# adrianstanea/UnitSpeech

Hardware: AMD Instinct MI355X
Metric: mel-frames/sec @ 50 diffusion steps, 80x1024 (higher is better)
Workload: dtype f32; 1 GPU; B=1 utterance(s)/GPU, 80x1024 mel, 50 diffusion steps, text+spk CFG (3 score evals/step), full-size decoder (119.1M params, synthetic weights), built-in Philox noise; batch_per_gpu=1, frames=1024, diffusion_steps=50, parallelism=utterance-sharded x1

## Files before the change

unitspeech_amd/csrc/attn.hip:

```cpp
#include "kernels.h"

namespace us {

typedef float f32x16 __attribute__((ext_vector_type(16)));
typedef float f32x4 __attribute__((ext_vector_type(4)));

constexpr int kChunk = 128;
constexpr int kQkvLd = 3 * kHidden;

__global__ __launch_bounds__(256) void attn_ctx_partial_kernel(const float* __restrict__ qkv, int n, float* __restrict__ part_ctx,
                                                               float* __restrict__ part_m, float* __restrict__ part_s, int nchunks) {
  const int b = blockIdx.y, chunk = blockIdx.x;
  const int lane = threadIdx.x & 63, h = threadIdx.x >> 6;
  const int c = lane & 31, hh = lane >> 5;
  const float* base = qkv + (long long)b * n * kQkvLd;
  const int r0 = chunk * kChunk;
  const float* kp = base + kHidden + h * kDimHead + c;
  const float* vp = base + 2 * kHidden + h * kDimHead + c;

  float kv[kChunk / 2];
  float m = -INFINITY;
#pragma unroll
  for (int j = 0; j < kChunk / 2; ++j) {
    int row = r0 + 2 * j + hh;
// ... 64 lines not shown
                                                              int per_split, float* __restrict__ ctx, float* __restrict__ split_ws) {
  const int b = blockIdx.x / kHeads, h = blockIdx.x % kHeads;
  const int d = threadIdx.x >> 5, e = threadIdx.x & 31;
  const float M = colM[(long long)b * kHidden + h * kDimHead + d], S = colS[(long long)b * kHidden + h * kDimHead + d];
  const int lo = blockIdx.y * per_split;
  int hi = lo + per_split;
  if (hi > nchunks) hi = nchunks;
  const float* pm = part_m + (long long)b * nchunks * kHidden + h * kDimHead + d;
  const float* pc = part_ctx + ((long long)b * nchunks * kHeads + h) * (kDimHead * kDimHead) + d * kDimHead + e;
  float acc0 = 0.f, acc1 = 0.f, acc2 = 0.f, acc3 = 0.f;
  int ch = lo;
  for (; ch + 4 <= hi; ch += 4) {
    float m0 = pm[(long long)ch * kHidden], m1 = pm[(long long)(ch + 1) * kHidden], m2 = pm[(long long)(ch + 2) * kHidden],
          m3 = pm[(long long)(ch + 3) * kHidden];
    float c0 = pc[(long long)ch * kHeads * 1024], c1 = pc[(long long)(ch + 1) * kHeads * 1024], c2 = pc[(long long)(ch + 2) * kHeads * 1024],
          c3 = pc[(long long)(ch + 3) * kHeads * 1024];
    acc0 = fmaf(expf(m0 - M), c0, acc0);
    acc1 = fmaf(expf(m1 - M), c1, acc1);
    acc2 = fmaf(expf(m2 - M), c2, acc2);
    acc3 = fmaf(expf(m3 - M), c3, acc3);
  }
  for (; ch < hi; ++ch) acc0 = fmaf(expf(pm[(long long)ch * kHidden] - M), pc[(long long)ch * kHeads * 1024], acc0);
  const float v = ((acc0 + acc1) + (acc2 + acc3)) / S;
  float* dst = (gridDim.y == 1 ? ctx : split_ws + (long long)blockIdx.y * gridDim.x * (kDimHead * kDimHead)) +
               ((long long)b * kHeads + h) * (kDimHead * kDimHead) + d * kDimHead + e;
  *dst = v;
}

__global__ __launch_bounds__(1024) void attn_ctx_reduce_kernel(const float* __restrict__ split_ws, int nsplit, long long slab,
                                                               float* __restrict__ ctx) {
  const long long i = blockIdx.x * 1024LL + threadIdx.x;
  float acc = split_ws[i];
  for (int k = 1; k < nsplit; ++k) acc += split_ws[i + k * slab];
  ctx[i] = acc;
}

hipError_t launch_attn_ctx_finalize(const float* part_ctx, const float* part_m, const float* part_s, int B, int nchunks,
                                    float* ctx, float* colM, float* colS, float* split_ws, hipStream_t s) {
  hipLaunchKernelGGL(attn_ctx_stats_kernel, dim3(B * kHeads), dim3(1024), 0, s, part_m, part_s, nchunks, colM, colS);
  int nsplit = (nchunks + 31) / 32;
  if (nsplit > kAttnMaxSplit) nsplit = kAttnMaxSplit;
  if (nsplit < 1 || !split_ws) nsplit = 1;
  const int per_split = (nchunks + nsplit - 1) / nsplit;
  nsplit = (nchunks + per_split - 1) / per_split;
  hipLaunchKernelGGL(attn_ctx_accum_kernel, dim3(B * kHeads, nsplit), dim3(1024), 0, s, part_ctx, part_m, colM, colS, nchunks, per_split, ctx,
                     split_ws);
  if (nsplit > 1)
    hipLaunchKernelGGL(attn_ctx_reduce_kernel, dim3(B * kHeads), dim3(1024), 0, s, split_ws, nsplit,
                       (long long)B * kHeads * kDimHead * kDimHead, ctx);
  return hipGetLastError();
}

__global__ __launch_bounds__(1024) void attn_merge_kernel(const float* __restrict__ part_ctx, const float* __restrict__ part_m,
                                                          const float* __restrict__ part_s, int nchunks, int per_range,
                                                          float* __restrict__ r_ctx, float* __restrict__ r_m, float* __restrict__ r_s) {
  __shared__ float s_m[64][kDimHead + 1];
  __shared__ float s_M[kDimHead], s_S[kDimHead];
  const int bh = blockIdx.y, b = bh / kHeads, h = bh % kHeads;
  const int d = threadIdx.x >> 5, e = threadIdx.x & 31;
  const int lo = blockIdx.x * per_range;
  const int hi = min(lo + per_range, nchunks);
  const float* pm = part_m + (long long)b * nchunks * kHidden + h * kDimHead;
  const float* ps = part_s + (long long)b * nchunks * kHidden + h * kDimHead;
  const float* pc = part_ctx + ((long long)b * nchunks * kHeads + h) * (kDimHead * kDimHead) + d * kDimHead + e;
  float M = -INFINITY;
  for (int ch = lo + d; ch < hi; ch += 32) M = fmaxf(M, pm[(long long)ch * kHidden + e]);
  s_m[d][e] = M;
  __syncthreads();
  if (d == 0) {
    float mm = s_m[0][e];
#pragma unroll
    for (int k = 1; k < 32; ++k) mm = fmaxf(mm, s_m[k][e]);
    s_M[e] = mm;
  }
  __syncthreads();
  {
    const float Mc = s_M[e];
    float S = 0.f;
    for (int ch = lo + d; ch < hi; ch += 32) S += ps[(long long)ch * kHidden + e] * expf(pm[(long long)ch * kHidden + e] - Mc);
    __syncthreads();
    s_m[d][e] = S;
    __syncthreads();
    if (d == 0) {
      float ss = 0.f;
#pragma unroll
      for (int k = 0; k < 32; ++k) ss += s_m[k][e];
      s_S[e] = ss;
    }
  }
  __syncthreads();
  const float Md = s_M[d];
  float acc0 = 0.f, acc1 = 0.f, acc2 = 0.f, acc3 = 0.f;
  for (int base = lo; base < hi; base += 64) {
    const int nb = min(64, hi - base);
    __syncthreads();
    for (int i = threadIdx.x; i < nb * kDimHead; i += 1024) {
      const int c = i >> 5, col = i & 31;
      s_m[c][col] = expf(pm[(long long)(base + c) * kHidden + col] - s_M[col]);
    }
    __syncthreads();
    int c = 0;
    for (; c + 8 <= nb; c += 8) {
      float v[8];
#pragma unroll
      for (int u = 0; u < 8; ++u) v[u] = pc[(long long)(base + c + u) * kHeads * 1024];
      acc0 = fmaf(s_m[c][d], v[0], acc0);     acc1 = fmaf(s_m[c + 1][d], v[1], acc1);
      acc2 = fmaf(s_m[c + 2][d], v[2], acc2); acc3 = fmaf(s_m[c + 3][d], v[3], acc3);
      acc0 = fmaf(s_m[c + 4][d], v[4], acc0); acc1 = fmaf(s_m[c + 5][d], v[5], acc1);
      acc2 = fmaf(s_m[c + 6][d], v[6], acc2); acc3 = fmaf(s_m[c + 7][d], v[7], acc3);
    }
    for (; c < nb; ++c) acc0 = fmaf(s_m[c][d], pc[(long long)(base + c) * kHeads * 1024], acc0);
  }
  (void)Md;
  const long long o = ((long long)blockIdx.x * gridDim.y + bh);
  r_ctx[o * 1024 + d * kDimHead + e] = (acc0 + acc1) + (acc2 + acc3);
  if (d == 0) { r_m[o * kDimHead + e] = s_M[e]; r_s[o * kDimHead + e] = s_S[e]; }
}

__global__ __launch_bounds__(1024) void attn_final_kernel(const float* __restrict__ r_ctx, const float* __restrict__ r_m,
                                                          const float* __restrict__ r_s, int nrange, float* __restrict__ ctx,
                                                          float* __restrict__ colM, float* __restrict__ colS, const float* __restrict__ wout,
                                                          float* __restrict__ weff, int C, int bk, int f16, unsigned* range_flag) {
  __shared__ float s_ctx[kDimHead][kDimHead + 1];
  __shared__ float s_w[16][kDimHead + 1];
  __shared__ float s_M[kDimHead], s_S[kDimHead];
  const int bh = blockIdx.x, b = bh / kHeads, h = bh % kHeads;
  const int d = threadIdx.x >> 5, e = threadIdx.x & 31;
  const int nbh = gridDim.x;
  const bool writer = blockIdx.y == 0;
  if (d == 0) {
    float M = -INFINITY;
    for (int r = 0; r < nrange; ++r) M = fmaxf(M, r_m[((long long)r * nbh + bh) * kDimHead + e]);
    float S = 0.f;
    for (int r = 0; r < nrange; ++r) {
      const float w = expf(r_m[((long long)r * nbh + bh) * kDimHead + e] - M);
      s_w[r][e] = w;
      S += r_s[((long long)r * nbh + bh) * kDimHead + e] * w;
    }
    s_M[e] = M; s_S[e] = S;
    if (writer) {
      colM[(long long)b * kHidden + h * kDimHead + e] = M;
      colS[(long long)b * kHidden + h * kDimHead + e] = S;
    }
  }
  __syncthreads();
  float acc = 0.f;
  for (int r = 0; r < nrange; ++r) acc = fmaf(s_w[r][d], r_ctx[((long long)r * nbh + bh) * 1024 + d * kDimHead + e], acc);
  const float v = acc / s_S[d];
  if (writer) ctx[((long long)b * kHeads + h) * 1024 + d * kDimHead + e] = v;
  if (!weff) return;
  s_ctx[d][e] = v;
  __syncthreads();
  const int dd = threadIdx.x & 31;
  bool over = false;
  const int co_end = min(C, ((int)blockIdx.y + 1) * 128);
  __shared__ float s_wo[128][kDimHead + 1];
  for (int i = threadIdx.x; i < 128 * kDimHead; i += 1024) {
    const int r = i >> 5, k = i & 31, co = blockIdx.y * 128 + r;
    s_wo[r][k] = co < C ? wout[(long long)co * kHidden + h * kDimHead + k] : 0.f;
  }
  __syncthreads();
  for (int co = blockIdx.y * 128 + (threadIdx.x >> 5); co < co_end; co += 32) {
    const float* w = s_wo[co - blockIdx.y * 128];
    float a2 = 0.f;
#pragma unroll
    for (int k = 0; k < kDimHead; ++k) a2 = fmaf(w[k], s_ctx[dd][k], a2);
    const int hd = h * kDimHead + dd;
    const long long o = (long long)b * C * kHidden + ((long long)(hd / bk) * C + co) * bk;
    if (!f16) {
      weff[o + hd % bk] = a2;
    } else {
      _Float16* w16 = reinterpret_cast<_Float16*>(weff + o);
      const int k = hd % 32;
      us_half hh_, ll_;
      split_f16x3(a2, hh_, ll_, over);
      w16[(k / 8) * 16 + k % 8] = hh_;
      w16[(k / 8) * 16 + 8 + k % 8] = ll_;
    }
  }
  range_report(range_flag, over, kRangeWeight);
}

hipError_t launch_attn_merge(const float* part_ctx, const float* part_m, const float* part_s, int B, int nchunks, float* ctx, float* colM,
                             float* colS, float* scratch, const float* wout, float* weff, int C, int bk, bool f16, hipStream_t s) {
  if (f16 && bk != 32) return hipErrorInvalidValue;
  int nrange = (nchunks + 63) / 64;
  if (nrange > kAttnMaxSplit) nrange = kAttnMaxSplit;
  if (nrange < 1) nrange = 1;
  const int per_range = (nchunks + nrange - 1) / nrange;
  nrange = (nchunks + per_range - 1) / per_range;
  const long long nbh = (long long)B * kHeads;
  float* r_ctx = scratch;
  float* r_m = r_ctx + (long long)kAttnMaxSplit * nbh * 1024;
  float* r_s = r_m + (long long)kAttnMaxSplit * nbh * kDimHead;
  hipLaunchKernelGGL(attn_merge_kernel, dim3(nrange, (unsigned)nbh), dim3(1024), 0, s, part_ctx, part_m, part_s, nchunks, per_range, r_ctx, r_m, r_s);
  hipLaunchKernelGGL(attn_final_kernel, dim3((unsigned)nbh, weff ? (unsigned)((C + 127) / 128) : 1u), dim3(1024), 0, s, r_ctx, r_m, r_s, nrange, ctx, colM, colS, wout, weff, C, bk,
                     f16 ? 1 : 0, current_range_flag());
  return hipGetLastError();
}

__global__ __launch_bounds__(256) void attn_wtotal_kernel(const float* __restrict__ ctx, const float* __restrict__ wout,
                                                          const float* __restrict__ wq, float* __restrict__ wtotal, int C, int bk, int f16,
                                                          unsigned* range_flag) {
  __shared__ __attribute__((aligned(16))) float s_T[kHidden][36];
  __shared__ float s_C[kHidden][33];
  __shared__ __attribute__((aligned(16))) float s_QW[kHidden * 36];
  const int b = blockIdx.y, k0 = blockIdx.x * 32, n0 = blockIdx.z * 32;
  const float* cx = ctx + (long long)b * kHeads * kDimHead * kDimHead;
  for (int i = threadIdx.x; i < kHidden * 32; i += 256) {
    s_C[i >> 5][i & 31] = cx[i];
    s_QW[(i >> 5) * 36 + (i & 31)] = wq[(long long)(i >> 5) * C + k0 + (i & 31)];
  }
  __syncthreads();
  for (int i = threadIdx.x; i < kHidden * 8; i += 256) {
    const int j = i >> 3, k4 = (i & 7) * 4;
    const int h = j / kDimHead, e = j % kDimHead;
    f32x4 acc = {0.f, 0.f, 0.f, 0.f};
#pragma unroll
    for (int d = 0; d < kDimHead; ++d) {
      const float c = s_C[h * kDimHead + d][e];
      const f32x4 q = *reinterpret_cast<const f32x4*>(&s_QW[(h * kDimHead + d) * 36 + k4]);
#pragma unroll
      for (int t = 0; t < 4; ++t) acc[t] = fmaf(c, q[t], acc[t]);
    }
    *reinterpret_cast<f32x4*>(&s_T[j][k4]) = acc;
  }
  __syncthreads();
  float* s_W = s_QW;
  for (int i = threadIdx.x; i < 32 * kHidden; i += 256) s_W[(i / kHidden) * (kHidden + 1) + i % kHidden] = wout[(long long)(n0 + i / kHidden) * kHidden + i % kHidden];
  __syncthreads();
  bool over = false;
  const int nl = threadIdx.x >> 3, g8 = threadIdx.x & 7;
  const int n = n0 + nl;
  f32x4 acc = {0.f, 0.f, 0.f, 0.f};
  for (int j = 0; j < kHidden; ++j) {
    const float wj = s_W[nl * (kHidden + 1) + j];
    const f32x4 tv = *reinterpret_cast<const f32x4*>(&s_T[j][g8 * 4]);
#pragma unroll
    for (int t = 0; t < 4; ++t) acc[t] = fmaf(wj, tv[t], acc[t]);
  }
  float* base = wtotal + (long long)b * C * C;
  if (f16) {
    typedef _Float16 half4_t __attribute__((ext_vector_type(4)));
    half4_t hi, lo;
#pragma unroll
    for (int t = 0; t < 4; ++t) {
      us_half h_, l_;
      split_f16x3(acc[t], h_, l_, over);
      hi[t] = h_;
      lo[t] = l_;
// ... 56 lines not shown
```

unitspeech_amd/csrc/decoder.hip:

```cpp
#include <hip/hip_runtime.h>

#include <cmath>
#include <cstdarg>
#include <cstdio>
#include <cstring>
#include <algorithm>
#include <map>
#include <memory>
#include <string>
#include <vector>

#include "../../include/unitspeech_hip.h"
#include "kernels.h"
#include "pack_f16.h"

using namespace us;

namespace {

thread_local std::string g_last_error;

struct DevBuf {
  float* p = nullptr;
  size_t n = 0;
// ... 42 lines not shown
  Slot *mlp_w, *mlp_b;
  ConvW c1, c2, res;
  Slot *g1, *b1, *g2, *b2;
  bool has_res = false;
  int index = 0;
};
struct AttnW {
  int dim, level;
  Slot* g;
  ConvW qkv;
  Slot *out_w, *out_b;
};
struct ResampleW {
  ConvW conv;
  int dim, level;
};

int pick_bk(int cin) { return (cin % 32 == 0) ? 32 : 16; }
constexpr const char* kWino4Default = "0,44,44,24";

}

namespace us {
void set_last_error(const char* msg) { g_last_error = msg ? msg : ""; }
}

struct us_decoder {
  us_config cfg{};
  int device = 0;
  std::vector<std::unique_ptr<Slot>> slots;
  std::map<std::string, Slot*> by_key;
  std::vector<int> C;
  struct Down { ResnetW r1, r2; AttnW a; bool has_ds; ResampleW ds; };
  struct Up { ResnetW r1, r2; AttnW a; ResampleW us; };
  std::vector<Down> downs;
  ResnetW mid1, mid2;
  AttnW mid_attn;
  std::vector<Up> ups;
  ConvW final_conv3;
  Slot *final_g, *final_b, *final_w1, *final_b1;
  Slot *text_uncon, *spk_uncon, *mlp0_w, *mlp0_b, *mlp2_w, *mlp2_b;
  int n_resnets = 0;
  int wino_min_level = 1;
  int wino4_level_form[8] = {0, 0, 0, 0, 0, 0, 0, 0};
  int wino_fuse = -1;
  bool wino_fuse_gn = true;
  int f16_tm = 0;
  int wgrad_side_streams = 1;
  std::vector<hipStream_t> wgrad_streams;
  std::vector<hipEvent_t> wgrad_events;
  bool training = false;
  float* zeros = nullptr;
  unsigned* range_flag = nullptr;
  unsigned* range_host = nullptr;
  bool exact = false;
  float* grad_scale = nullptr;
  CopyEnt* grad_tab_dev = nullptr;
  static constexpr size_t kLinJobs = 64;
  LinJob *lin_tab_dev = nullptr, *lin_tab_bwd_dev = nullptr;
  std::vector<CopyEnt> pending_copies;
  std::vector<PackJob> pending_packs;
  PackJob* pack_tab_dev = nullptr;
  static constexpr size_t kStageBytes = 64 << 10;
  CopyEnt* copy_tab_dev = nullptr;
  CopyEnt* copy_tab_host[4] = {nullptr, nullptr, nullptr, nullptr};
  static constexpr int kCaptureTabs = 32;
  size_t copy_tab_capture_bytes[kCaptureTabs] = {};
  CopyEnt* copy_tab_capture[kCaptureTabs] = {};
  int copy_tab_capture_used = 0;
  hipEvent_t copy_tab_ev[4] = {nullptr, nullptr, nullptr, nullptr};
  int copy_tab_i = 0;
  size_t copy_tab_cap = 0;
  std::map<uint64_t, std::shared_ptr<void>> tapes;
  uint64_t tape_serial = 0;
  static constexpr size_t kMaxTapes = 16;
  std::string err;

  struct ProfRec { hipEvent_t a, b; double flops; int kind; int f16 = 0; };
  bool prof_enabled = false;
  bool prof_active = false;
  std::vector<ProfRec> prof_pending;
  std::vector<hipEvent_t> prof_pool;
  double prof_conv_ms = 0, prof_conv_flops = 0, prof_eval_ms = 0;
  long long prof_conv_launches = 0, prof_evals = 0;
  double prof_f16_ms = 0, prof_f16_flops = 0;
  long long prof_f16_launches = 0;
  hipEvent_t prof_event() {
    if (!prof_pool.empty()) { hipEvent_t e = prof_pool.back(); prof_pool.pop_back(); return e; }
    hipEvent_t e = nullptr;
    (void)hipEventCreate(&e);
    return e;
  }

  int fail(int code, const char* fmt, ...) {
    char buf[512];
    va_list ap;
    va_start(ap, fmt);
    vsnprintf(buf, sizeof buf, fmt, ap);
    va_end(ap);
    err = buf;
    g_last_error = buf;
    return code;
  }

  Slot* add(const std::string& key, std::vector<int64_t> shape, Kind kind = Kind::RAW, int bk = 0) {
    slots.emplace_back(new Slot());
// ... 522 lines not shown
    g.stats = st1; g.gamma = r.g1->buf.p; g.beta = r.b1->buf.p; g.temb = tproj;
    g.mask = e.mask; g.mask_ld = e.T; g.mask_step = 1 << l; g.mask_bmod = e.Bm;
    CK(conv3x3_wino(e, r.c2, S1, r.cout, l, S2, r.cout, st2, &g));
  } else {
    if (direct_presplit(e, r.c2, r.cout, out_ld) && out != in) {
      CK(gn_apply(e, S1, l, r.cout, st1, r.g1, r.b1, tproj, nullptr, 0, false, true, out, r.cout, true));
      CK(conv3x3(e, r.c2, out, r.cout, l, S2, r.cout, st2, true));
    } else {
      CK(gn_apply(e, S1, l, r.cout, st1, r.g1, r.b1, tproj, nullptr, 0, false, true, S1, r.cout));
      CK(conv3x3(e, r.c2, S1, r.cout, l, S2, r.cout, st2));
    }
  }
  if (R) {
    CK(gn_apply(e, S2, l, r.cout, st2, r.g2, r.b2, nullptr, R, r.cout, false, mask_out, out, out_ld, false, split_out));
  } else if (r.has_res) {
    CK(gn_apply(e, S2, l, r.cout, st2, r.g2, r.b2, nullptr, nullptr, 0, false, false, out, out_ld));
    CK(conv1x1(e, r.res, in, in_ld, l, mask_out, out, out_ld, out, out_ld, nullptr, nullptr, 0, nullptr, in_split));
  } else {
    CK(gn_apply(e, S2, l, r.cout, st2, r.g2, r.b2, nullptr, in, in_ld, false, mask_out, out, out_ld, false, split_out));
  }
  return hipSuccess;
}

inline bool next_takes_split_copy(EvalCtx& e, const ResnetW& r2) {
  return !e.h->exact && !r2.has_res && !r2.first && direct_presplit(e, r2.c1, r2.c1.cin, r2.c1.cin) &&
         r2.c1.cin == r2.cout;
}

inline bool resnet_takes_split(EvalCtx& e, const ResnetW& r) {
  return !r.first && r.has_res && !(r.c1.w->wino.p && e.b->wino_v) && r.c1.w->direct_f16 && r.res.w->direct_f16;
}

hipError_t attention(EvalCtx& e, const AttnW& at, const float* in, int in_ld, float* out, int out_ld, bool out_split = false) {
  Buffers& b = *e.b;
  const int l = at.level;
  const int n = (e.h->cfg.n_feats >> l) * (e.T >> l);
  const int nch = attn_nchunks(n);
  float* qkv = b.QKV[l];
  int q_ld = 3 * kHidden;
  int nparts = nch;
  if (at.qkv.w->qkv_rows.p && at.qkv.w->q_raw.p && b.wtotal && l == 0 && at.dim <= kWtotalMaxC && at.dim % 32 == 0) {
    const int H = e.h->cfg.n_feats >> l, W = e.T >> l;
    const int nch64 = (n + 63) / 64;
    ConvArgs a = base_args(e, at.qkv, in, in_ld, H, W, qkv, kHidden, H, W);
    a.Cout = 2 * kHidden;
    a.wt_rows = 3 * kHidden;
    a.wt = at.qkv.w->qkv_rows.p + (size_t)kHidden * at.qkv.w->bk;
    a.ntaps = 1;
    a.set_tap(0, 0, 0, 0);
    a.attn_part_ctx = b.part_ctx; a.attn_part_m = b.part_m; a.attn_part_s = b.part_s; a.attn_nchunks = nch64;
    a.attn_q_cols = 0;
    CK(run_conv(e, a));
    const bool f16 = !e.h->exact;
    CK(launch_attn_merge(b.part_ctx, b.part_m, b.part_s, e.Bp, nch64, b.ctx, b.colM, b.colS, b.ctx_split, at.out_w->buf.p, nullptr, at.dim,
                         pick_bk(kHidden), f16, e.s));
    const int bkc = pick_bk(at.dim);
    CK(launch_attn_wtotal(b.ctx, at.out_w->buf.p, at.qkv.w->q_raw.p, b.wtotal, e.Bp, at.dim, bkc, f16, e.s));
    ConvW tot;
    tot.cin = at.dim; tot.cout = at.dim;
    Slot tmp;
    tmp.bk = bkc; tmp.buf.p = b.wtotal; tmp.direct_f16 = f16;
    tot.w = &tmp; tot.b = nullptr;
    return conv1x1(e, tot, in, in_ld, l, true, out, out_ld, in, in_ld, at.g->buf.p, b.wtotal, (long long)at.dim * at.dim, at.out_b->buf.p,
                   false, out_split);
  }
  if (at.qkv.w->qkv_rows.p) {
    const int H = e.h->cfg.n_feats >> l, W = e.T >> l;
    const int nch64 = (n + 63) / 64;
    q_ld = kHidden;
    ConvArgs a = base_args(e, at.qkv, in, in_ld, H, W, qkv, q_ld, H, W);
    a.wt = at.qkv.w->qkv_rows.p;
    a.ntaps = 1;
    a.set_tap(0, 0, 0, 0);
    a.attn_part_ctx = b.part_ctx; a.attn_part_m = b.part_m; a.attn_part_s = b.part_s; a.attn_nchunks = nch64;
    a.attn_q_cols = kHidden;
    CK(run_conv(e, a));
    nparts = nch64;
  } else {
    CK(conv1x1(e, at.qkv, in, in_ld, l, false, qkv, 3 * kHidden, nullptr, 0, nullptr, nullptr, 0, nullptr));
    CK(launch_attn_ctx_partial(qkv, e.Bp, n, b.part_ctx, b.part_m, b.part_s, nch, e.s));
  }
  const int bk = pick_bk(kHidden);
  const bool f16 = !e.h->exact;
  CK(launch_attn_merge(b.part_ctx, b.part_m, b.part_s, e.Bp, nparts, b.ctx, b.colM, b.colS, b.ctx_split, at.out_w->buf.p, b.weff, at.dim, bk,
                       f16, e.s));
  ConvW eff;
  eff.cin = kHidden; eff.cout = at.dim;
  Slot tmp;
  tmp.bk = bk; tmp.buf.p = b.weff; tmp.direct_f16 = f16;
  eff.w = &tmp; eff.b = nullptr;
  return conv1x1(e, eff, qkv, q_ld, l, true, out, out_ld, in, in_ld, at.g->buf.p, b.weff, (long long)at.dim * kHidden,
                 at.out_b->buf.p, false, out_split);
}

int upload_bytes(us_decoder* h, const void* src, size_t nbytes, void* dev, hipStream_t st);

inline int proj_jobs(us_decoder* h, std::vector<LinJob>& jobs, std::vector<const ResnetW*>& blocks) {
  jobs.clear();
  blocks.clear();
  int o0 = 0;
  auto add = [&](const ResnetW& r) {
    LinJob j;
    memset(&j, 0, sizeof j);
    j.W = r.mlp_w->buf.p; j.bias = r.mlp_b->buf.p; j.o0 = o0; j.cout = r.cout; j.out_ld = r.cout;
    jobs.push_back(j);
    blocks.push_back(&r);
    o0 += r.cout;
  };
  for (auto& d : h->downs) { add(d.r1); add(d.r2); }
  add(h->mid1); add(h->mid2);
  for (auto& u : h->ups) { add(u.r1); add(u.r2); }
  return o0;
}

hipError_t time_embedding(EvalCtx& e, const float* t, const float* spk) {
  us_decoder* h = e.h;
  Buffers& b = *e.b;
  const int dim = h->cfg.dim, S = h->cfg.spk_emb_dim, td = dim + S;
  CK(launch_pos_emb(t, b.posemb, e.Bp, dim, h->cfg.pe_scale, e.s));
  CK(launch_linear(b.posemb, dim, h->mlp0_w->buf.p, h->mlp0_b->buf.p, b.mlp_h, 4 * dim, e.Bp, dim, 4 * dim, false, e.s));
  CK(launch_linear(b.mlp_h, 4 * dim, h->mlp2_w->buf.p, h->mlp2_b->buf.p, b.temb, td, e.Bp, 4 * dim, dim, true, e.s));
  CK(launch_copy_rows(spk, S, e.Bp, b.temb + dim, td, e.Bp, S, e.s));
  std::vector<LinJob> jobs;
  std::vector<const ResnetW*> blocks;
  const int total = proj_jobs(h, jobs, blocks);
  if (h->lin_tab_dev && jobs.size() <= us_decoder::kLinJobs) {
    for (size_t i = 0; i < jobs.size(); ++i) jobs[i].out = b.tproj + b.tproj_off[blocks[i]->index];
    if (upload_bytes(h, jobs.data(), jobs.size() * sizeof(LinJob), h->lin_tab_dev, e.s) != US_OK) return hipErrorUnknown;
    return launch_linear_multi(h->lin_tab_dev, (int)jobs.size(), total, b.temb, td, e.Bp, td, true, e.s);
  }
  auto proj = [&](const ResnetW& r) {
    return launch_linear(b.temb, td, r.mlp_w->buf.p, r.mlp_b->buf.p, b.tproj + b.tproj_off[r.index], r.cout, e.Bp, td, r.cout, true,
                         e.s);
  };
  for (auto& d : h->downs) { CK(proj(d.r1)); CK(proj(d.r2)); }
  CK(proj(h->mid1)); CK(proj(h->mid2));
  for (auto& u : h->ups) { CK(proj(u.r1)); CK(proj(u.r2)); }
// ... 245 lines not shown
  if (h->cfg.n_feats % q != 0) return h->fail(US_EINVAL, "n_feats=%d is not divisible by %d", h->cfg.n_feats, q);
  return US_OK;
}

}

extern "C" {

int us_decoder_create(us_handle* out, const us_config* cfg) { return us_decoder_create_ex(out, cfg, 0u); }

int us_decoder_create_ex(us_handle* out, const us_config* cfg, unsigned flags) {
  if (!out || !cfg) { g_last_error = "null argument"; return US_EINVAL; }
  if (flags & ~(unsigned)US_CREATE_EXACT_FP32) { g_last_error = "unknown creation flag"; return US_EINVAL; }
  if (cfg->n_mults < 1 || cfg->n_mults > 6 || cfg->dim < 16 || cfg->dim % 16 != 0 || cfg->n_feats <= 0 || cfg->spk_emb_dim <= 0 ||
      cfg->spk_emb_dim % 4 != 0) {
    g_last_error = "unsupported configuration (dim must be a multiple of 16, 1 <= n_mults <= 6)";
    return US_EINVAL;
  }
  for (int i = 0; i < cfg->n_mults; ++i) {
    int c = cfg->dim * cfg->dim_mults[i];
    int cg = c / kGroups;
    if (cfg->dim_mults[i] < 1 || c % 16 != 0 || (cg & (cg - 1)) != 0) {
      g_last_error = "unsupported dim_mults (channels/8 must be a power of two)";
      return US_EINVAL;
    }
  }
  std::unique_ptr<us_decoder> h(new us_decoder());
  h->cfg = *cfg;
  if (hipGetDevice(&h->device) != hipSuccess) { g_last_error = "no HIP device"; return US_EHIP; }
  hipError_t e = conv_igemm_init();
  if (e != hipSuccess) { g_last_error = std::string("conv_igemm_init: ") + hipGetErrorString(e); return US_EHIP; }
  h->exact = (flags & US_CREATE_EXACT_FP32) != 0;
  if (const char* wl = getenv("US_WINO_MIN_LEVEL")) h->wino_min_level = atoi(wl);
  if (const char* wf = getenv("US_WINO_FUSE")) h->wino_fuse = atoi(wf) != 0 ? 1 : 0;
  if (const char* wf = getenv("US_WINO_FUSE_GN")) h->wino_fuse_gn = atoi(wf) != 0;
  if (const char* wt = getenv("US_F16_TM")) h->f16_tm = atoi(wt) == 64 || atoi(wt) == 128 || atoi(wt) == 256 ? atoi(wt) : 0;
  if (const char* ws = getenv("US_WGRAD_STREAM")) h->wgrad_side_streams = atoi(ws) < 0 ? 0 : (atoi(ws) > Tape::kSideMax ? Tape::kSideMax : atoi(ws));
  {
    const char* w4 = getenv("US_WINO4");
    std::string spec = w4 ? w4 : kWino4Default;
    size_t pos = 0;
    for (int l = 0; l < 8 && pos <= spec.size(); ++l) {
      const size_t comma = spec.find(',', pos);
      const std::string tok = spec.substr(pos, comma == std::string::npos ? std::string::npos : comma - pos);
      const int f = tok.empty() ? 0 : atoi(tok.c_str());
      h->wino4_level_form[l] = wino4_form_ok(f) ? f : 0;
      if (comma == std::string::npos) break;
      pos = comma + 1;
    }
    if (h->exact)
      for (int l = 0; l < 8; ++l) h->wino4_level_form[l] = 0;
  }
  h->build();
  if (hipMalloc(reinterpret_cast<void**>(&h->range_flag), 256) != hipSuccess || hipMemset(h->range_flag, 0, 256) != hipSuccess ||
      hipHostMalloc(reinterpret_cast<void**>(&h->range_host), 256) != hipSuccess ||
      hipMalloc(reinterpret_cast<void**>(&h->grad_scale), 256) != hipSuccess) {
    g_last_error = "allocation of the range word failed";
    return US_EHIP;
  }
  *h->range_host = 0u;
  {
    int max_cin = 2 * h->C.back();
    for (int c : h->C) if (2 * c > max_cin) max_cin = 2 * c;
    size_t zb = ((size_t)max_cin + 64) * sizeof(float);
    if (hipMalloc(reinterpret_cast<void**>(&h->zeros), zb) != hipSuccess || hipMemset(h->zeros, 0, zb) != hipSuccess) {
      g_last_error = "hipMalloc failed for the zero page";
      return US_EHIP;
    }
  }
  for (auto& s : h->slots) {
    bool ok = true;
    s->buf.n = numel(s->shape);
    if (!s->want_wino) {
      ok = hipMalloc(reinterpret_cast<void**>(&s->buf.p), s->buf.n * sizeof(float)) == hipSuccess;
      if (ok && (s->kind != Kind::RAW || s->dg_as_1x1)) {
        s->dg.n = s->buf.n;
        ok = hipMalloc(reinterpret_cast<void**>(&s->dg.p), s->dg.n * sizeof(float)) == hipSuccess;
      }
    }
    if (ok && s->is_qkv) {
      s->qkv_rows.n = s->buf.n;
      ok = hipMalloc(reinterpret_cast<void**>(&s->qkv_rows.p), s->qkv_rows.n * sizeof(float)) == hipSuccess;
      s->q_raw.n = (size_t)kHidden * s->shape[1];
      ok = ok && hipMalloc(reinterpret_cast<void**>(&s->q_raw.p), s->q_raw.n * sizeof(float)) == hipSuccess;
    }
    if (ok && s->want_wino) {
      s->wino.n = s->wino_dg.n = (size_t)16 * s->shape[0] * s->shape[1];
      ok = hipMalloc(reinterpret_cast<void**>(&s->wino.p), s->wino.n * sizeof(float)) == hipSuccess &&
           hipMalloc(reinterpret_cast<void**>(&s->wino_dg.p), s->wino_dg.n * sizeof(float)) == hipSuccess;
    }
    if (ok && s->dg.p && !h->exact) {
      const long long kk = s->kind == Kind::CONVT_IOHW ? s->shape[1] : s->shape[0];
      s->dg_f16 = kk % 32 == 0;
    }
    if (ok && !s->want_wino && s->kind != Kind::RAW && !h->exact) {
      const long long cin = s->kind == Kind::CONV_OIHW ? s->shape[1] : s->shape[0];
      s->direct_f16 = cin % 32 == 0;
    }
    if (ok && s->want_wino && !h->exact) {
      s->wino_f16 = s->shape[1] % 32 == 0;
      s->wino_dg_f16 = s->shape[0] % 32 == 0;
    }
    constexpr int kWino4MinK = 256;
    if (ok && s->want_wino && s->wino_f16 && s->level >= 0 && s->level < 8 && wino4_form_ok(h->wino4_level_form[s->level]) && s->shape[0] % 8 == 0 &&
        s->shape[1] >= kWino4MinK) {
      s->wino4_form = h->wino4_level_form[s->level];
      s->wino4.n = (size_t)wino4_freqs(s->wino4_form) * s->shape[0] * s->shape[1];
      ok = hipMalloc(reinterpret_cast<void**>(&s->wino4.p), s->wino4.n * sizeof(float)) == hipSuccess;
    }
    if (!ok) {
      g_last_error = "hipMalloc failed for weight store";
      for (auto& t : h->slots) { if (t->buf.p) (void)hipFree(t->buf.p); if (t->dg.p) (void)hipFree(t->dg.p); if (t->wino.p) (void)hipFree(t->wino.p); if (t->wino_dg.p) (void)hipFree(t->wino_dg.p); if (t->wino4.p) (void)hipFree(t->wino4.p); if (t->qkv_rows.p) (void)hipFree(t->qkv_rows.p); if (t->q_raw.p) (void)hipFree(t->q_raw.p); }
      return US_EHIP;
// ... 500 lines not shown
```

unitspeech_amd/csrc/kernels.h:

```cpp
#pragma once
#include <hip/hip_runtime.h>
#include <stdint.h>

namespace us {

#if defined(__HIPCC__)
__device__ __forceinline__ float mul_rn(float a, float b) {
#pragma clang fp contract(off)
  return a * b;
}
__device__ __forceinline__ float add_rn(float a, float b) {
#pragma clang fp contract(off)
  return a + b;
}
__device__ __forceinline__ float sub_rn(float a, float b) {
#pragma clang fp contract(off)
  return a - b;
}
#endif

constexpr float kF16Over = 65520.f;
enum : unsigned {
  kRangeAct = 1u,
  kRangeWeight = 2u,
// ... 94 lines not shown
  double t = 0.0;
#pragma unroll
  for (int i = 0; i < kStatSlots; ++i) t += p[i];
  return t;
}
#endif
inline int qkv_src_row(int cp) {
  if (cp < kHidden) return cp;
  const int t = cp - kHidden, h = t >> 6, w = t & 63;
  return (w < kDimHead ? kHidden : 2 * kHidden) + h * kDimHead + (w & (kDimHead - 1));
}
hipError_t launch_conv_igemm(const ConvArgs& a, hipStream_t s);
hipError_t conv_igemm_init();

hipError_t launch_pack_conv_weight(const float* src, float* dst, int Cout, int Cin, int KH, int KW, bool oihw, int bk,
                                   hipStream_t s, bool qkv_rows = false);
hipError_t launch_pack_conv_weight_f16(const float* src, float* dst, int Cout, int Cin, int KH, int KW, bool oihw, hipStream_t s,
                                       bool qkv_rows = false);

hipError_t launch_first_conv(const float* in2, const float* w3, const float* b3, const float* w1, const float* b1, float* y,
                             float* r, double* stats, int Bp, int F, int T, int C, hipStream_t s);
hipError_t launch_stack_inputs(const float* x, int Bx, const float* mu, int Bmu, int n_text_uncond, const float* mu_feat,
                               const float* mask, int Bm, float* in2, int Bp, int F, int T, hipStream_t s);

hipError_t launch_gn_stats(const float* y, int ld, int B, int n, int C, double* stats, hipStream_t s);
struct GnApplyArgs {
  const float* y; int y_ld;
  const double* stats;
  const float* gamma; const float* beta;
  const float* mask; int mask_ld, mask_step, mask_bmod;
  const float* temb; int temb_ld;
  const float* res; int res_ld; int res_masked;
  const float* res2_in; const float* res2_w; const float* res2_b;
  int post_mask;
  unsigned* range_flag;
  int out_split;
  float* out; int out_ld;
  float* out2; int out2_ld;
  int B, H, W, C;
};
hipError_t launch_gn_apply(const GnApplyArgs& a, hipStream_t s);
hipError_t launch_final_conv(const float* h, int ld, const float* w, const float* b0, const float* mask, int mask_ld,
                             int mask_bmod, float* out, int B, int H, int W, int C, hipStream_t s, const double* stats = nullptr,
                             const float* gamma = nullptr, const float* beta = nullptr);

hipError_t launch_attn_ctx_partial(const float* qkv, int B, int n, float* part_ctx, float* part_m, float* part_s, int nchunks,
                                   hipStream_t s);
constexpr int kAttnMaxSplit = 16;
hipError_t launch_attn_ctx_finalize(const float* part_ctx, const float* part_m, const float* part_s, int B, int nchunks,
                                    float* ctx, float* colM, float* colS, float* split_ws, hipStream_t s);
hipError_t launch_attn_wtotal(const float* ctx, const float* wout, const float* wq, float* wtotal, int B, int C, int bk, bool f16, hipStream_t s);
hipError_t launch_attn_weff(const float* ctx, const float* wout , float* weff, int B, int C, int bk, hipStream_t s,
                            bool f16 = false);
inline size_t attn_merge_scratch_floats(int B) { return (size_t)kAttnMaxSplit * B * kHeads * (kDimHead * kDimHead + 2 * kDimHead); }
hipError_t launch_attn_merge(const float* part_ctx, const float* part_m, const float* part_s, int B, int nchunks, float* ctx, float* colM,
                             float* colS, float* scratch, const float* wout, float* weff, int C, int bk, bool f16, hipStream_t s);
inline int attn_nchunks(int n) { return (n + 127) / 128; }

hipError_t launch_linear(const float* in, int in_ld, const float* W, const float* bias, float* out, int out_ld, int rows,
                         int in_dim, int out_dim, bool mish_in, hipStream_t s);
hipError_t launch_pos_emb(const float* t, float* emb, int rows, int dim, float scale, hipStream_t s);
hipError_t launch_copy_rows(const float* src, int src_ld, int src_rows, float* dst, int dst_ld, int rows, int n, hipStream_t s);
hipError_t launch_fill(float* dst, float value, int n, hipStream_t s);
struct CopyEnt { const float* src; float* dst; long long n; };
hipError_t launch_copy_table(const CopyEnt* tab_dev, int n_entries, hipStream_t s);
hipError_t launch_scale_table(const CopyEnt* tab_dev, int n_entries, const float* scale_dev, hipStream_t s);
hipError_t launch_pow2_scale(const float* x, long long n, int target_log2, float* out2, hipStream_t s);
hipError_t launch_scale(const float* x, const float* scalar_dev, float* out, long long n, hipStream_t s);
hipError_t launch_l2_normalize(const float* src, float* dst, int n, hipStream_t s);

struct SamplerArgs {
  const float* xt; const float* score; const float* noise; const float* mask;
  float* out;
  int B, F, T, mode;
  float w_text, w_spk;
  float c0, c1, c2, c3, c4, c5;
  unsigned long long seed; long long utt0; int step;
};
hipError_t launch_sampler_update(const SamplerArgs& a, hipStream_t s);
hipError_t launch_mul_mask(const float* x, const float* mask, float* out, int B, int F, int T, hipStream_t s);
hipError_t launch_finish_mel(const float* x, const float* mask, float* out, int B, int F, int T, const float* mel_range_host, hipStream_t s);
hipError_t launch_first_conv_dgrad(const float* gy, const float* gr, const float* w3, const float* w1, const float* mask, float* gmu,
                                   float* gx, int B, int F, int T, int C, hipStream_t s);
void set_last_error(const char* msg);
hipError_t launch_fill_normal(float* out, size_t n, unsigned long long seed, unsigned long long key, hipStream_t s);

struct WgradArgs {
  const float* gy; int gy_ld;
  const float* x; int x_ld;
  float* gw; long long gw_bstride;
  int B, Hin, Win, Cin, Hout, Wout, Cout;
  int Hs, Ws, oy0, ox0, ostep, istride, ntaps;
  int chunk;
  int vchunk;
  int exact;
  const float* gy_amax;
  int overwrite;
  unsigned long long dy_bits, dx_bits, wtap_bits;
  void set_tap(int i, int dy, int dx, int wtap) {
    dy_bits |= (unsigned long long)(dy + 8) << (4 * i);
    dx_bits |= (unsigned long long)(dx + 8) << (4 * i);
    wtap_bits |= (unsigned long long)wtap << (4 * i);
  }
};
hipError_t launch_wgrad(const WgradArgs& a, hipStream_t s);
hipError_t launch_wgrad_amax(const float* g, int ld, long long rows, int C, float* out, hipStream_t s);
bool launch_wgrad_single_writer(const WgradArgs& a);
hipError_t launch_unpack_wgrad(const float* src, float* dst, int Cout, int Cin, int taps, bool oihw, hipStream_t s, const float* scale = nullptr);
hipError_t launch_pack_dgrad_weight(const float* src, float* dst, int Cout, int Cin, int KH, int KW, bool oihw, int bk, hipStream_t s);
// ... 84 lines not shown
```

unitspeech_amd/csrc/train_host.inc:

```

inline hipError_t zero_f32(float* p, size_t n, hipStream_t s) {
  while (n > 0) {
    const size_t chunk = n > (size_t)1 << 30 ? (size_t)1 << 30 : n;
    hipError_t e = launch_fill(p, 0.f, (int)chunk, s);
    if (e != hipSuccess) return e;
    p += chunk;
    n -= chunk;
  }
  return hipSuccess;
}
inline hipError_t zero_f64(double* p, size_t n, hipStream_t s) { return zero_f32(reinterpret_cast<float*>(p), 2 * n, s); }

struct ResT {
  const ResnetW* w = nullptr;
  const float* x = nullptr; int x_ld = 0;
  float *y1 = nullptr, *h1 = nullptr, *y2 = nullptr, *out = nullptr, *r0 = nullptr;
  int out_ld = 0;
  double *st1 = nullptr, *st2 = nullptr;
  bool mask_out = false;
};
struct AttT {
  const AttnW* w = nullptr;
  const float* x = nullptr; int x_ld = 0;
  float *qkv = nullptr, *ctx = nullptr, *colM = nullptr, *colS = nullptr, *weff = nullptr, *out = nullptr;
// ... 141 lines not shown
  tp.gsum = A.alloc<double>((size_t)(2 * h->n_resnets + 1) * B * kGroups * 2);
  tp.gctx_stride = B * kHeads * kDimHead * kDimHead;
  tp.gctx = A.alloc<float>(tp.gctx_stride * (tp.att.size() ? tp.att.size() : 1));
  size_t tsum = 0;
  for (size_t i = 0; i < tp.fb.tproj_off.size(); ++i) tsum = tp.fb.tproj_off[i] > tsum ? tp.fb.tproj_off[i] : tsum;
  tp.gtproj = A.alloc<float>(tsum + B * (size_t)cmax);
  tp.gtemb = A.alloc<float>(B * (h->cfg.dim + h->cfg.spk_emb_dim));
  tp.gmlp_h = A.alloc<float>(B * 4 * h->cfg.dim);
  tp.amax = A.alloc<float>(Tape::kAmaxSlots);
  tp.zero_lo = reinterpret_cast<float*>(tp.gsum);
  tp.zero_floats = (size_t)(reinterpret_cast<char*>(tp.amax + Tape::kAmaxSlots) - reinterpret_cast<char*>(tp.gsum)) / sizeof(float);
  tp.red_partials = A.alloc<double>((size_t)kRedBlocks * tp.att.size() + (size_t)final_bwd_blocks(Bp, F, T, h->C[0]) * B);
  tp.mask_copy = A.alloc<float>(B * (size_t)T);
  tp.gscaled = A.alloc<float>(B * (size_t)F * T);
}

inline hipError_t resnet_train(EvalCtx& e, Tape& tp, const ResnetW& r, const float* in, int in_ld, bool mask_out) {
  ResT& t = tp.res[r.index];
  t.x = in; t.x_ld = in_ld; t.mask_out = mask_out;
  const int l = r.level;
  const float* tproj = tp.fb.tproj + tp.fb.tproj_off[r.index];
  CK(conv3x3(e, r.c1, in, in_ld, l, t.y1, r.cout, t.st1));
  if (r.c2.w->wino.p && e.b->wino_v && gn_wino_input_supported(r.cout)) {
    WinoGnArgs g;
    memset(&g, 0, sizeof g);
    g.stats = t.st1; g.gamma = r.g1->buf.p; g.beta = r.b1->buf.p; g.temb = tproj;
    g.mask = e.mask; g.mask_ld = e.T; g.mask_step = 1 << l; g.mask_bmod = e.Bm;
    g.h_out = t.h1;
    CK(conv3x3_wino(e, r.c2, t.y1, r.cout, l, t.y2, r.cout, t.st2, &g));
  } else {
    CK(gn_apply(e, t.y1, l, r.cout, t.st1, r.g1, r.b1, tproj, nullptr, 0, false, true, t.h1, r.cout));
    CK(conv3x3(e, r.c2, t.h1, r.cout, l, t.y2, r.cout, t.st2));
  }
  if (r.has_res) {
    CK(gn_apply(e, t.y2, l, r.cout, t.st2, r.g2, r.b2, nullptr, nullptr, 0, false, false, t.out, t.out_ld));
    CK(conv1x1(e, r.res, in, in_ld, l, mask_out, t.out, t.out_ld, t.out, t.out_ld, nullptr, nullptr, 0, nullptr));
  } else {
    CK(gn_apply(e, t.y2, l, r.cout, t.st2, r.g2, r.b2, nullptr, in, in_ld, false, mask_out, t.out, t.out_ld));
  }
  return hipSuccess;
}

inline hipError_t attention_train(EvalCtx& e, Tape& tp, AttT& t, const float* in, int in_ld) {
  const AttnW& at = *t.w;
  Buffers& b = tp.fb;
  t.x = in; t.x_ld = in_ld;
  const int l = at.level;
  const int n = (e.h->cfg.n_feats >> l) * (e.T >> l);
  const int nch = attn_nchunks(n);
  CK(conv1x1(e, at.qkv, in, in_ld, l, false, t.qkv, 3 * kHidden, nullptr, 0, nullptr, nullptr, 0, nullptr));
  CK(launch_attn_ctx_partial(t.qkv, e.Bp, n, b.part_ctx, b.part_m, b.part_s, nch, e.s));
  const int bk = pick_bk(kHidden);
  const bool f16 = !e.h->exact;
  CK(launch_attn_merge(b.part_ctx, b.part_m, b.part_s, e.Bp, nch, t.ctx, t.colM, t.colS, b.ctx_split, at.out_w->buf.p, t.weff, at.dim, bk, f16,
                       e.s));
  ConvW eff;
  eff.cin = kHidden; eff.cout = at.dim;
  Slot tmp;
  tmp.bk = bk; tmp.buf.p = t.weff; tmp.direct_f16 = f16;
  eff.w = &tmp; eff.b = nullptr;
  return conv1x1(e, eff, t.qkv, 3 * kHidden, l, true, t.out, t.out_ld, in, in_ld, at.g->buf.p, t.weff, (long long)at.dim * kHidden,
                 at.out_b->buf.p, false, false, t.o_pre, at.dim);
}

inline hipError_t train_forward(us_decoder* h, Tape& tp, hipStream_t s, const float* x, const float* mu, const float* mask, const float* t,
                                const float* spk, float* out) {
  const int L = h->cfg.n_mults, F = h->cfg.n_feats, T = tp.T, Bp = tp.Bp;
  CK(hipMemcpyAsync(tp.mask_copy, mask, sizeof(float) * (size_t)Bp * T, hipMemcpyDeviceToDevice, s));
  mask = tp.mask_copy;
  EvalCtx e{h, s, &tp.fb, Bp, T, mask, Bp};
  e.splitk_by_batch = 1;
  tp.mask = mask; tp.Bm = Bp;
  CK(zero_f64(tp.stats_all, tp.stats_all_count, s));
  CK(time_embedding(e, t, spk));
  CK(launch_stack_inputs(x, Bp, mu, Bp, 0, h->text_uncon->buf.p, mask, Bp, tp.fb.in2, Bp, F, T, s));
  const float* cur = nullptr;
  int cur_ld = 0;
  size_t ai = 0, di = 0;
  for (int l = 0; l < L; ++l) {
    auto& d = h->downs[l];
    const int c = h->C[l];
    if (l == 0) {
      const ResnetW& r = d.r1;
      ResT& rt = tp.res[r.index];
      rt.x = tp.fb.in2; rt.x_ld = 2; rt.mask_out = true;
      CK(launch_first_conv(tp.fb.in2, r.c1.w->buf.p, r.c1.b->buf.p, r.res.w->buf.p, r.res.b->buf.p, rt.y1, rt.r0, rt.st1, Bp, F, T, c, s));
      CK(gn_apply(e, rt.y1, 0, c, rt.st1, r.g1, r.b1, tp.fb.tproj + tp.fb.tproj_off[r.index], nullptr, 0, false, true, rt.h1, c));
      CK(conv3x3(e, r.c2, rt.h1, c, 0, rt.y2, c, rt.st2));
      CK(gn_apply(e, rt.y2, 0, c, rt.st2, r.g2, r.b2, nullptr, rt.r0, c, false, true, rt.out, rt.out_ld));
    } else {
      CK(resnet_train(e, tp, d.r1, cur, cur_ld, true));
    }
    ResT& r1t = tp.res[d.r1.index];
    CK(resnet_train(e, tp, d.r2, r1t.out, r1t.out_ld, false));
    ResT& r2t = tp.res[d.r2.index];
    AttT& at = tp.att[ai++];
    CK(attention_train(e, tp, at, r2t.out, r2t.out_ld));
    if (d.has_ds) {
      CvT& c = tp.downs[di++];
      c.x = at.out; c.x_ld = at.out_ld;
      CK(conv_down(e, *c.w, at.out, at.out_ld, l, c.out, c.out_ld));
      cur = c.out; cur_ld = c.out_ld;
    } else {
      cur = at.out; cur_ld = at.out_ld;
    }
  }
  CK(resnet_train(e, tp, h->mid1, cur, cur_ld, false));
// ... 580 lines not shown
```

Measured before the change: 3197 mel-frames/s.

## Fuse attention merge and final reduction via last-block atomic counter

Merges the attention range-merge kernel and the final kernel into one launch. Each range block publishes partial results, then an atomic counter per (batch-head, tile) selects the last-arriving block, which does the cross-range softmax combine and the weff projection tile. The aim is to save one kernel launch and the gap between the two kernels on every attention call. The cost is threadfence and atomic traffic, a counter buffer carved from the range-flag allocation, and the z dimension now duplicating merge work per output tile.

```diff
diff --git a/unitspeech_amd/csrc/attn.hip b/unitspeech_amd/csrc/attn.hip
--- a/unitspeech_amd/csrc/attn.hip
+++ b/unitspeech_amd/csrc/attn.hip
@@ -140,12 +140,16 @@
 }
 
 __global__ __launch_bounds__(1024) void attn_merge_kernel(const float* __restrict__ part_ctx, const float* __restrict__ part_m,
-                                                          const float* __restrict__ part_s, int nchunks, int per_range,
-                                                          float* __restrict__ r_ctx, float* __restrict__ r_m, float* __restrict__ r_s) {
+                                                          const float* __restrict__ part_s, int nchunks, int per_range, float* r_ctx,
+                                                          float* r_m, float* r_s, float* __restrict__ ctx, float* __restrict__ colM,
+                                                          float* __restrict__ colS, const float* __restrict__ wout, float* __restrict__ weff,
+                                                          int C, int bk, int f16, unsigned* range_flag, unsigned* counters) {
   __shared__ float s_m[64][kDimHead + 1];
   __shared__ float s_M[kDimHead], s_S[kDimHead];
+  __shared__ unsigned s_last;
   const int bh = blockIdx.y, b = bh / kHeads, h = bh % kHeads;
   const int d = threadIdx.x >> 5, e = threadIdx.x & 31;
+  const int nrange = gridDim.x, nbh = gridDim.y, zt = gridDim.z, z = blockIdx.z;
   const int lo = blockIdx.x * per_range;
   const int hi = min(lo + per_range, nchunks);
   const float* pm = part_m + (long long)b * nchunks * kHidden + h * kDimHead;
@@ -177,7 +181,6 @@
     }
   }
   __syncthreads();
-  const float Md = s_M[d];
   float acc0 = 0.f, acc1 = 0.f, acc2 = 0.f, acc3 = 0.f;
   for (int base = lo; base < hi; base += 64) {
     const int nb = min(64, hi - base);
@@ -199,78 +202,94 @@
     }
     for (; c < nb; ++c) acc0 = fmaf(s_m[c][d], pc[(long long)(base + c) * kHeads * 1024], acc0);
   }
-  (void)Md;
-  const long long o = ((long long)blockIdx.x * gridDim.y + bh);
+  const long long slab0 = (long long)z * nrange * nbh + bh;
+  const long long o = slab0 + (long long)blockIdx.x * nbh;
   r_ctx[o * 1024 + d * kDimHead + e] = (acc0 + acc1) + (acc2 + acc3);
   if (d == 0) { r_m[o * kDimHead + e] = s_M[e]; r_s[o * kDimHead + e] = s_S[e]; }
-}
-
-__global__ __launch_bounds__(1024) void attn_final_kernel(const float* __restrict__ r_ctx, const float* __restrict__ r_m,
-                                                          const float* __restrict__ r_s, int nrange, float* __restrict__ ctx,
-                                                          float* __restrict__ colM, float* __restrict__ colS, const float* __restrict__ wout,
-                                                          float* __restrict__ weff, int C, int bk, int f16, unsigned* range_flag) {
+
+  if (nrange > 1) {
+    __threadfence();
+    __syncthreads();
+    if (threadIdx.x == 0) {
+      unsigned* cnt = counters + (long long)bh * zt + z;
+      const unsigned seen = atomicAdd(cnt, 1u);
+      const bool last = seen == (unsigned)nrange - 1u;
+      if (last) atomicExch(cnt, 0u);
+      s_last = last ? 1u : 0u;
+    }
+    __syncthreads();
+    if (!s_last) return;
+    __threadfence();
+  } else {
+    __syncthreads();
+  }
+
   __shared__ float s_ctx[kDimHead][kDimHead + 1];
-  __shared__ float s_w[16][kDimHead + 1];
-  __shared__ float s_M[kDimHead], s_S[kDimHead];
-  const int bh = blockIdx.x, b = bh / kHeads, h = bh % kHeads;
-  const int d = threadIdx.x >> 5, e = threadIdx.x & 31;
-  const int nbh = gridDim.x;
-  const bool writer = blockIdx.y == 0;
+  __shared__ float s_w[kAttnMaxSplit][kDimHead + 1];
+  __shared__ float s_wo[128][kDimHead + 1];
+  const bool writer = z == 0;
   if (d == 0) {
-    float M = -INFINITY;
-    for (int r = 0; r < nrange; ++r) M = fmaxf(M, r_m[((long long)r * nbh + bh) * kDimHead + e]);
+    float Mx = -INFINITY;
+    for (int r = 0; r < nrange; ++r) Mx = fmaxf(Mx, r_m[(slab0 + (long long)r * nbh) * kDimHead + e]);
     float S = 0.f;
     for (int r = 0; r < nrange; ++r) {
-      const float w = expf(r_m[((long long)r * nbh + bh) * kDimHead + e] - M);
+      const float w = expf(r_m[(slab0 + (long long)r * nbh) * kDimHead + e] - Mx);
       s_w[r][e] = w;
-      S += r_s[((long long)r * nbh + bh) * kDimHead + e] * w;
-    }
-    s_M[e] = M; s_S[e] = S;
+      S += r_s[(slab0 + (long long)r * nbh) * kDimHead + e] * w;
+    }
+    s_M[e] = Mx; s_S[e] = S;
     if (writer) {
-      colM[(long long)b * kHidden + h * kDimHead + e] = M;
+      colM[(long long)b * kHidden + h * kDimHead + e] = Mx;
       colS[(long long)b * kHidden + h * kDimHead + e] = S;
     }
   }
   __syncthreads();
   float acc = 0.f;
-  for (int r = 0; r < nrange; ++r) acc = fmaf(s_w[r][d], r_ctx[((long long)r * nbh + bh) * 1024 + d * kDimHead + e], acc);
+  for (int r = 0; r < nrange; ++r) acc = fmaf(s_w[r][d], r_ctx[(slab0 + (long long)r * nbh) * 1024 + d * kDimHead + e], acc);
   const float v = acc / s_S[d];
   if (writer) ctx[((long long)b * kHeads + h) * 1024 + d * kDimHead + e] = v;
   if (!weff) return;
   s_ctx[d][e] = v;
-  __syncthreads();
   const int dd = threadIdx.x & 31;
   bool over = false;
-  const int co_end = min(C, ((int)blockIdx.y + 1) * 128);
-  __shared__ float s_wo[128][kDimHead + 1];
-  for (int i = threadIdx.x; i < 128 * kDimHead; i += 1024) {
-    const int r = i >> 5, k = i & 31, co = blockIdx.y * 128 + r;
-    s_wo[r][k] = co < C ? wout[(long long)co * kHidden + h * kDimHead + k] : 0.f;
-  }
-  __syncthreads();
-  for (int co = blockIdx.y * 128 + (threadIdx.x >> 5); co < co_end; co += 32) {
-    const float* w = s_wo[co - blockIdx.y * 128];
-    float a2 = 0.f;
-#pragma unroll
-    for (int k = 0; k < kDimHead; ++k) a2 = fmaf(w[k], s_ctx[dd][k], a2);
-    const int hd = h * kDimHead + dd;
-    const long long o = (long long)b * C * kHidden + ((long long)(hd / bk) * C + co) * bk;
-    if (!f16) {
-      weff[o + hd % bk] = a2;
-    } else {
-      _Float16* w16 = reinterpret_cast<_Float16*>(weff + o);
-      const int k = hd % 32;
-      us_half hh_, ll_;
-      split_f16x3(a2, hh_, ll_, over);
-      w16[(k / 8) * 16 + k % 8] = hh_;
-      w16[(k / 8) * 16 + 8 + k % 8] = ll_;
+  const int ntiles = (C + 127) / 128;
+  for (int tile = z; tile < ntiles; tile += zt) {
+    const int co_end = min(C, (tile + 1) * 128);
+    __syncthreads();
+    for (int i = threadIdx.x; i < 128 * kDimHead; i += 1024) {
+      const int r = i >> 5, k = i & 31, co = tile * 128 + r;
+      s_wo[r][k] = co < C ? wout[(long long)co * kHidden + h * kDimHead + k] : 0.f;
+    }
+    __syncthreads();
+    for (int co = tile * 128 + (threadIdx.x >> 5); co < co_end; co += 32) {
+      const float* w = s_wo[co - tile * 128];
+      float a2 = 0.f;
+#pragma unroll
+      for (int k = 0; k < kDimHead; ++k) a2 = fmaf(w[k], s_ctx[dd][k], a2);
+      const int hd = h * kDimHead + dd;
+      const long long oo = (long long)b * C * kHidden + ((long long)(hd / bk) * C + co) * bk;
+      if (!f16) {
+        weff[oo + hd % bk] = a2;
+      } else {
+        _Float16* w16 = reinterpret_cast<_Float16*>(weff + oo);
+        const int k = hd % 32;
+        us_half hh_, ll_;
+        split_f16x3(a2, hh_, ll_, over);
+        w16[(k / 8) * 16 + k % 8] = hh_;
+        w16[(k / 8) * 16 + 8 + k % 8] = ll_;
+      }
     }
   }
   range_report(range_flag, over, kRangeWeight);
 }
 
+int attn_merge_zt(int nrange, long long nbh, int ntiles) {
+  return ntiles > 1 && (long long)nrange * ntiles <= kAttnMaxSplit && nbh * ntiles <= kAttnCounterWords ? ntiles : 1;
+}
+
 hipError_t launch_attn_merge(const float* part_ctx, const float* part_m, const float* part_s, int B, int nchunks, float* ctx, float* colM,
-                             float* colS, float* scratch, const float* wout, float* weff, int C, int bk, bool f16, hipStream_t s) {
+                             float* colS, float* scratch, unsigned* counters, const float* wout, float* weff, int C, int bk, bool f16,
+                             hipStream_t s) {
   if (f16 && bk != 32) return hipErrorInvalidValue;
   int nrange = (nchunks + 63) / 64;
   if (nrange > kAttnMaxSplit) nrange = kAttnMaxSplit;
@@ -278,12 +297,13 @@
   const int per_range = (nchunks + nrange - 1) / nrange;
   nrange = (nchunks + per_range - 1) / per_range;
   const long long nbh = (long long)B * kHeads;
+  const int zt = attn_merge_zt(nrange, nbh, weff ? (C + 127) / 128 : 1);
+  if (nrange > 1 && (!counters || nbh * zt > kAttnCounterWords)) return hipErrorInvalidValue;
   float* r_ctx = scratch;
   float* r_m = r_ctx + (long long)kAttnMaxSplit * nbh * 1024;
   float* r_s = r_m + (long long)kAttnMaxSplit * nbh * kDimHead;
-  hipLaunchKernelGGL(attn_merge_kernel, dim3(nrange, (unsigned)nbh), dim3(1024), 0, s, part_ctx, part_m, part_s, nchunks, per_range, r_ctx, r_m, r_s);
-  hipLaunchKernelGGL(attn_final_kernel, dim3((unsigned)nbh, weff ? (unsigned)((C + 127) / 128) : 1u), dim3(1024), 0, s, r_ctx, r_m, r_s, nrange, ctx, colM, colS, wout, weff, C, bk,
-                     f16 ? 1 : 0, current_range_flag());
+  hipLaunchKernelGGL(attn_merge_kernel, dim3(nrange, (unsigned)nbh, zt), dim3(1024), 0, s, part_ctx, part_m, part_s, nchunks, per_range, r_ctx,
+                     r_m, r_s, ctx, colM, colS, wout, weff, C, bk, f16 ? 1 : 0, current_range_flag(), counters);
   return hipGetLastError();
 }
 
diff --git a/unitspeech_amd/csrc/decoder.hip b/unitspeech_amd/csrc/decoder.hip
--- a/unitspeech_amd/csrc/decoder.hip
+++ b/unitspeech_amd/csrc/decoder.hip
@@ -118,6 +118,7 @@
   bool training = false;
   float* zeros = nullptr;
   unsigned* range_flag = nullptr;
+  unsigned* attn_count = nullptr;
   unsigned* range_host = nullptr;
   bool exact = false;
   float* grad_scale = nullptr;
@@ -746,7 +747,7 @@
     a.attn_q_cols = 0;
     CK(run_conv(e, a));
     const bool f16 = !e.h->exact;
-    CK(launch_attn_merge(b.part_ctx, b.part_m, b.part_s, e.Bp, nch64, b.ctx, b.colM, b.colS, b.ctx_split, at.out_w->buf.p, nullptr, at.dim,
+    CK(launch_attn_merge(b.part_ctx, b.part_m, b.part_s, e.Bp, nch64, b.ctx, b.colM, b.colS, b.ctx_split, e.h->attn_count, at.out_w->buf.p, nullptr, at.dim,
                          pick_bk(kHidden), f16, e.s));
     const int bkc = pick_bk(at.dim);
     CK(launch_attn_wtotal(b.ctx, at.out_w->buf.p, at.qkv.w->q_raw.p, b.wtotal, e.Bp, at.dim, bkc, f16, e.s));
@@ -776,7 +777,7 @@
   }
   const int bk = pick_bk(kHidden);
   const bool f16 = !e.h->exact;
-  CK(launch_attn_merge(b.part_ctx, b.part_m, b.part_s, e.Bp, nparts, b.ctx, b.colM, b.colS, b.ctx_split, at.out_w->buf.p, b.weff, at.dim, bk,
+  CK(launch_attn_merge(b.part_ctx, b.part_m, b.part_s, e.Bp, nparts, b.ctx, b.colM, b.colS, b.ctx_split, e.h->attn_count, at.out_w->buf.p, b.weff, at.dim, bk,
                        f16, e.s));
   ConvW eff;
   eff.cin = kHidden; eff.cout = at.dim;
@@ -1128,13 +1129,15 @@
       for (int l = 0; l < 8; ++l) h->wino4_level_form[l] = 0;
   }
   h->build();
-  if (hipMalloc(reinterpret_cast<void**>(&h->range_flag), 256) != hipSuccess || hipMemset(h->range_flag, 0, 256) != hipSuccess ||
+  if (hipMalloc(reinterpret_cast<void**>(&h->range_flag), 256 + kAttnCounterWords * sizeof(unsigned)) != hipSuccess ||
+      hipMemset(h->range_flag, 0, 256 + kAttnCounterWords * sizeof(unsigned)) != hipSuccess ||
       hipHostMalloc(reinterpret_cast<void**>(&h->range_host), 256) != hipSuccess ||
       hipMalloc(reinterpret_cast<void**>(&h->grad_scale), 256) != hipSuccess) {
     g_last_error = "allocation of the range word failed";
     return US_EHIP;
   }
   *h->range_host = 0u;
+  h->attn_count = h->range_flag + 64;
   {
     int max_cin = 2 * h->C.back();
     for (int c : h->C) if (2 * c > max_cin) max_cin = 2 * c;
diff --git a/unitspeech_amd/csrc/kernels.h b/unitspeech_amd/csrc/kernels.h
--- a/unitspeech_amd/csrc/kernels.h
+++ b/unitspeech_amd/csrc/kernels.h
@@ -170,9 +170,12 @@
 hipError_t launch_attn_wtotal(const float* ctx, const float* wout, const float* wq, float* wtotal, int B, int C, int bk, bool f16, hipStream_t s);
 hipError_t launch_attn_weff(const float* ctx, const float* wout , float* weff, int B, int C, int bk, hipStream_t s,
                             bool f16 = false);
+constexpr int kAttnCounterWords = 16384;
 inline size_t attn_merge_scratch_floats(int B) { return (size_t)kAttnMaxSplit * B * kHeads * (kDimHead * kDimHead + 2 * kDimHead); }
+int attn_merge_zt(int nrange, long long nbh, int ntiles);
 hipError_t launch_attn_merge(const float* part_ctx, const float* part_m, const float* part_s, int B, int nchunks, float* ctx, float* colM,
-                             float* colS, float* scratch, const float* wout, float* weff, int C, int bk, bool f16, hipStream_t s);
+                             float* colS, float* scratch, unsigned* counters, const float* wout, float* weff, int C, int bk, bool f16,
+                             hipStream_t s);
 inline int attn_nchunks(int n) { return (n + 127) / 128; }
 
 hipError_t launch_linear(const float* in, int in_ld, const float* W, const float* bias, float* out, int out_ld, int rows,
diff --git a/unitspeech_amd/csrc/train_host.inc b/unitspeech_amd/csrc/train_host.inc
--- a/unitspeech_amd/csrc/train_host.inc
+++ b/unitspeech_amd/csrc/train_host.inc
@@ -217,7 +217,7 @@
   CK(launch_attn_ctx_partial(t.qkv, e.Bp, n, b.part_ctx, b.part_m, b.part_s, nch, e.s));
   const int bk = pick_bk(kHidden);
   const bool f16 = !e.h->exact;
-  CK(launch_attn_merge(b.part_ctx, b.part_m, b.part_s, e.Bp, nch, t.ctx, t.colM, t.colS, b.ctx_split, at.out_w->buf.p, t.weff, at.dim, bk, f16,
+  CK(launch_attn_merge(b.part_ctx, b.part_m, b.part_s, e.Bp, nch, t.ctx, t.colM, t.colS, b.ctx_split, e.h->attn_count, at.out_w->buf.p, t.weff, at.dim, bk, f16,
                        e.s));
   ConvW eff;
   eff.cin = kHidden; eff.cout = at.dim;
```

Measured after the change: 3090 mel-frames/s. 3.3% lower.
